# heiheishuang/MuDG

Hardware: AMD Instinct MI355X
Metric: DDIM denoise steps/sec, MDM1024 576x1024x16f (CFG: 2 UNet forwards + fused update per step, per clip) (higher is better)
Workload: dtype bf16; 1 GPU; MDM1024 latents (B=1,4,16,72,128) + c_concat 8ch, context (B,333,1024), 50-step uniform_trailing DDIM schedule, cfg 7.5, guidance_rescale 0.7, eta 1.0, v-prediction, dynamic rescale; clips_per_gpu=1, parallelism=clip-DP x1 (no in-step collective), launch=hipGraph replay of each UNet pass (cond+uncond batched)

## Files before the change

include/mudg_hip.h:

```cpp
#ifndef MUDG_HIP_H
#define MUDG_HIP_H

#include <stdint.h>

#ifdef __cplusplus
extern "C" {
#endif

#define MUDG_OK          0
#define MUDG_EINVAL     -1
#define MUDG_ELAUNCH    -2
#define MUDG_EUNSUPPORTED -3

int mudg_version(void);
int mudg_operand_dtype(void);
const char* mudg_last_error(void);

typedef struct MudgGemmDesc {
    const void* X;
    const void* X2;
    const void* W;
    void*       Y;
    const float* bias;
    const float* gbias;
// ... 3 lines not shown
    int csplit;
    int batch;
    int64_t sX, sW, sY, sR;
    int rows_per_group;
    int out_fp32;
    int res_fp32;
    int geglu;
    int act;
    float alpha;
    int mode;
    int Hin, Win, Hout, Wout, Cin, stride, upsample;
    int pad;
    int korder;
    int T, HW;
    float* stats;
    int subpixel;
    void* Y8; void* S8;
    int ldy8, lds8;
} MudgGemmDesc;
int mudg_gemm(const MudgGemmDesc* d, void* stream);
int mudg_gemm_stats_rows(const MudgGemmDesc* d);
int mudg_conv_subpixel_ok(const MudgGemmDesc* d);
int mudg_gemm_stream_ok(const MudgGemmDesc* d);

typedef struct MudgAttnDesc {
    const void* Q; const void* K; const void* Vt; void* O;
    int F, heads, Nq, Nk;
    int ldq, ldk, ldvt, ldo;
    int64_t svt;
    int kv_div;
    float scale;
    int accumulate;
    const void* K2; const void* Vt2;
    int Nk2, ldk2, ldvt2, kv_div2;
    int64_t svt2;
    const void* Q8; const void* K8; const void* Qs; const void* Ks;
    int ldq8, ldk8, ldqs, ldks;
    int q_prescaled;
    float* Lse;
} MudgAttnDesc;
int mudg_attention(const MudgAttnDesc* d, void* stream);
int mudg_quantize_mxfp8(const void* X, int ldx, int64_t rows, int cols, void* Y8, int ldy, void* S, int lds, void* stream);

int mudg_temporal_attention(const void* QKV, void* O, int B, int T, int HW, int heads,
                            int ldqkv, int ldo, float scale, void* stream);
int mudg_temporal_self_attention_ok(int T, int HW, int heads, int C, int64_t ldx, int64_t ldw, int64_t ldo);
// ... 240 lines not shown
```

mudg_amd/csrc/gemm.hip:

```cpp
#include "gemm_shared.h"
#include <cstdlib>
#include <cmath>
#include <type_traits>

namespace {


template <int NWAVES_, int NI_>
struct Geo {
    static constexpr int NWAVES = NWAVES_, NI = NI_, MI = 2, WN = 2, WM = NWAVES_ / 2;
    static constexpr int NTH = NWAVES * 64;
    static constexpr int BM = WM * MI * 32, BN = WN * NI * 32;
    static constexpr int XI = BM / NWAVES / 8, WI = BN / NWAVES / 8;
    static constexpr int TILE_X = BM * LDSLD, TILE_W = BN * LDSLD;
    static constexpr int STGLD = BN + 4;
    static constexpr bool WIDE = NWAVES > 4;
    static constexpr int WSTRIDE = !WIDE ? NI : (NI & 1 ? 1 : 2);
    static constexpr int nioff(int ni) { return !WIDE ? ni : (NI & 1 ? 2 * ni : 4 * (ni >> 1) + (ni & 1)); }
};
using G128 = Geo<4, 2>;
using G320 = Geo<8, 5>;
using G256 = Geo<8, 4>;

template <typename G> constexpr int stage_elems(bool fast) { return (fused_planes(fast) ? PLANES : 1) * (G::TILE_X + G::TILE_W); }
// ... 722 lines not shown
}
namespace {

template <typename G, int MODE, bool FAST, bool SB = false>
int launch(const MudgGemmDesc& d, int vflags, hipStream_t s) {
    const h16* zp = zero_page();
    if (!zp) MUDG_FAIL(MUDG_ELAUNCH, "gemm: could not allocate the zero page");
    constexpr int smem = smem_main<G>(FAST, SB);
    if (const int rc = mudg_lds_opt_in<&gemm_kernel<G, MODE, FAST, SB>>(smem + PHI_BYTES, "gemm")) return rc;
    const int tiles = ((d.M + G::BM - 1) / G::BM) * ((d.N + G::BN - 1) / G::BN);
    dim3 grid(tiles, 1, d.batch);
    const float* phi = d.geglu ? mudg_phi_table() : nullptr;
    hipLaunchKernelGGL((gemm_kernel<G, MODE, FAST, SB>), grid, dim3(G::NTH), smem + (phi ? PHI_BYTES : 0), s, d, vflags, zp, phi);
    return mudg_check_launch("mudg_gemm");
}

struct GemmSwitches {
    int fast = mudg_variant("GEMM_FAST", 1), sb = mudg_variant("GEMM_SB", 1), persist = mudg_variant("GEMM_PERSIST", 1);
    int wide = mudg_variant("GEMM_WIDE", 2), xshare = mudg_variant("CONV_XSHARE", 1);
    int w288 = mudg_variant("GEMM_W288", 1), w288p = mudg_variant("GEMM_W288P", 1), w288q = mudg_variant("GEMM_W288Q", 0);
    int h144 = mudg_variant("GEMM_H144", 1), h144pf = mudg_variant("GEMM_H144PF", 1);
    int h144delay = mudg_variant("GEMM_H144DELAY", 0) | (mudg_variant("GEMM_H144ABL", 0) << 16) | (mudg_variant("GEMM_H144PRIO", 1) ? 0 : 1 << 20);
    int w160 = mudg_variant("GEMM_W160", 1), w160defer = mudg_variant("GEMM_W160DEFER", 1);
    int stream = mudg_variant("GEMM_STREAM", 1);
};

bool fast_ok(const MudgGemmDesc& d, const GemmSwitches& sw) {
    if (!sw.fast) return false;
    const int cin = d.mode == 0 ? d.K : d.Cin;
    if ((d.K & 63) || (cin & 63) || (d.csplit & 63)) return false;
    if (d.mode == 1 && (d.upsample || d.Hout * d.Wout <= 0)) return false;
    const int64_t ld = d.X2 && d.ldx2 > d.ldx ? d.ldx2 : d.ldx;
    int64_t rel = 255, soff = (int64_t)cin * 2 + (PLANES > 1 ? ld * 2 : 0);
    if (d.mode == 1) {
        rel = (int64_t)(255 / (d.Hout * d.Wout) + 2) * d.Hin * d.Win;
        soff += (int64_t)(2 * d.Win + 2) * ld * 2;
    } else if (d.mode == 2) {
        soff += (int64_t)2 * d.HW * ld * 2;
        if (d.korder) rel = (int64_t)(d.T - 1) * d.HW + 8;
    }
    const int64_t lim = (int64_t)1 << 31;
    return rel * ld * 2 + 128 + soff + 16 < lim && (int64_t)(255 + (PLANES > 1)) * d.ldw * 2 + (int64_t)d.K * 2 + 144 < lim;
}

int access_flags(const MudgGemmDesc& d) {
    int vflags = 0;
    const int ybytes = d.out_fp32 == KIND_F32 ? 4 : 2;
// ... 88 lines not shown

bool wgemm288_ok(const MudgGemmDesc& d, int vflags, const GemmSwitches& sw) {
    if (!sw.w288 || !wgemm_eligible(d, vflags, WBM)) return false;
    if (sw.w288 == 2) return true;
    if (PLANES == 1 && d.geglu && half_height_ok(d, sw)) return true;
    const int S = d.mode == 1 ? d.Hout * d.Wout : d.HW;
    if (S <= 0 || S % WBM != 0) return false;
    if (d.mode != 0 || PLANES == 2) return true;
    if (d.geglu && d.K < 640) return w288_persistent_grid(d, sw) > 0;
    return true;
}

int stream_grid(const MudgGemmDesc& d, int vflags, const GemmSwitches& sw) {
    if (PLANES != 1 || !sw.stream) return 0;
    if (d.mode != 0 || d.K != 320 || (d.N != 320 && d.N != 640) || d.X2 || d.gbias || d.geglu || d.stats) return 0;
    if (sw.stream == 3 && d.N != 320) return 0;
    if (d.out_fp32 == KIND_F32 || (d.R && d.res_fp32 == KIND_F32)) return 0;
    if (!wgemm_eligible(d, vflags, WBM)) return 0;
    if (sw.stream != 2 && !(sw.w288 == 1 && sw.w288p != 2 && sw.w288q != 2 && wgemm288_ok(d, vflags, sw))) return 0;
    const int n = mudg_cu_count(), slices = d.N / 320;
    return n <= 0 ? 0 : ((n < 8 ? 8 : n) / (8 * slices)) * 8 * slices;
}

bool w160_ok(const MudgGemmDesc& d, int vflags, const GemmSwitches& sw) {
    if (!sw.w160 || !wgemm_eligible(d, vflags, QBM)) return false;
    if (sw.w160 == 2) return true;
    const int S = d.mode == 1 ? d.Hout * d.Wout : d.HW;
    if (S <= 0 || S % QBM != 0) return false;
    if (S < 640 || d.geglu) return false;
    if (d.mode != 0) return true;
    return d.K >= 1280;
}

void normalise_desc(MudgGemmDesc& d) {
    if (d.batch < 1) d.batch = 1;
    if (!d.X2) d.csplit = d.mode == 0 ? d.K : d.Cin;
    if (d.alpha == 0.f) d.alpha = 1.f;
}

GemmPlan gemm_plan(const MudgGemmDesc& d) {
    const GemmSwitches sw;
    GemmPlan p{};
    p.vflags = access_flags(d);
    if (d.mode == 2 && d.korder && fast_ok(d, sw)) p.vflags |= VF_TM;
    if (sw.xshare && d.mode == 1 && d.korder && !d.subpixel && !d.upsample && d.stride == 1 && d.pad == 1 && d.Hin == d.Hout && d.Win == d.Wout &&
        d.K == 9 * d.Cin && (d.Cin & 63) == 0)
        p.vflags |= VF_XS;
    p.rows = 128;
    if (const int sg = stream_grid(d, p.vflags, sw); sg > 0) {
        p.rows = WBM;
        p.kernel = GK_STREAM;
        p.grid = sg;
    } else if (PLANES <= 2 && wgemm288_ok(d, p.vflags, sw)) {
        p.rows = WBM;
        if (PLANES == 1 && sw.w288p != 2 && sw.w288q == 2) {
            p.kernel = GK_W288Q;
        } else if (PLANES == 1 && d.geglu && half_height_ok(d, sw)) {
            p.kernel = GK_H144;
            p.pf = sw.h144pf != 0;
            p.delay = sw.h144delay;
        } else if (PLANES == 1 && (p.grid = w288_persistent_grid(d, sw)) > 0) {
            p.kernel = GK_W288P;
        } else {
            p.kernel = GK_W288;
        }
    } else if (PLANES == 1 && w160_ok(d, p.vflags, sw)) {
        p.rows = QBM;
        p.kernel = GK_W160;
        p.rs = !d.R ? 0 : ((d.res_fp32 != KIND_F32 && sw.w160defer) ? 2 : 1);
    } else if (fast_ok(d, sw)) {
        if (PLANES == 1 && (p.ni = use_wide(d, sw)) != 0) {
            p.kernel = GK_WIDE;
        } else if (persistent_ok(d, p.vflags, sw)) {
            p.kernel = GK_PERSIST;
            p.wgs = persistent_wgs(d, sw);
// ... 2 lines not shown
        }
    } else {
        p.kernel = GK_GENERIC;
    }
    return p;
}

}

extern "C" int mudg_gemm_stats_rows(const MudgGemmDesc* dp) {
    if (!dp) return 128;
    MudgGemmDesc d = *dp;
    if (d.out_fp32 < 0 || d.out_fp32 > 2 || d.res_fp32 < 0 || d.res_fp32 > 2 || d.mode < 0 || d.mode > 2) return 128;
    normalise_desc(d);
    return gemm_plan(d).rows;
}

extern "C" int mudg_gemm_stream_ok(const MudgGemmDesc* dp) {
    if (!dp) return 0;
    MudgGemmDesc d = *dp;
    if (d.out_fp32 < 0 || d.out_fp32 > 2 || d.res_fp32 < 0 || d.res_fp32 > 2 || d.mode < 0 || d.mode > 2) return 0;
    normalise_desc(d);
    return gemm_plan(d).kernel == GK_STREAM ? 1 : 0;
}

extern "C" int mudg_conv_subpixel_ok(const MudgGemmDesc* dp) {
    if (!dp) return 0;
    MudgGemmDesc d = *dp;
    if (d.mode != 1 || !d.subpixel || d.batch != 4 || d.stride != 1 || d.pad != 1 || d.upsample || !d.korder) return 0;
    if (d.X2 || d.R || d.gbias || d.stats || d.geglu || d.sX != 0 || d.sY != 0) return 0;
    if (d.Hout != d.Hin || d.Wout != d.Win || d.K != 4 * d.Cin || (d.Cin & 63)) return 0;
    d.csplit = d.Cin;
    return fast_ok(d, GemmSwitches{}) ? 1 : 0;
}

extern "C" int mudg_gemm(const MudgGemmDesc* dp, void* stream) {
    MUDG_REQUIRE(dp, "mudg_gemm: null descriptor");
    MudgGemmDesc d = *dp;
    MUDG_REQUIRE(d.X && d.W && d.Y, "mudg_gemm: null X/W/Y");
    MUDG_REQUIRE(d.M > 0 && d.N > 0 && d.K > 0, "mudg_gemm: empty problem M=%d N=%d K=%d", d.M, d.N, d.K);
    MUDG_REQUIRE(d.mode >= 0 && d.mode <= 2, "mudg_gemm: mode %d", d.mode);
    MUDG_REQUIRE((d.K & 7) == 0, "mudg_gemm: K=%d must be a multiple of 8", d.K);
    MUDG_REQUIRE(d.ldx % (8 * PLANES) == 0 && d.ldw % (8 * PLANES) == 0, "mudg_gemm: ldx=%d ldw=%d must be multiples of %d", d.ldx, d.ldw, 8 * PLANES);
    MUDG_REQUIRE(aligned16(d.X) && aligned16(d.W), "mudg_gemm: X/W must be 16-byte aligned");
    MUDG_REQUIRE((d.sX & 7) == 0 && (d.sW & 7) == 0, "mudg_gemm: batch strides must be multiples of 8");
    normalise_desc(d);
// ... 41 lines not shown
    }
    const GemmPlan plan = gemm_plan(d);
    hipStream_t s = reinterpret_cast<hipStream_t>(stream);
    const int fam = d.mode == 0 ? MUDG_FAM_GEMM : (d.mode == 1 ? MUDG_FAM_CONV : MUDG_FAM_TCONV);
    const int slot = mudg_prof_begin(fam, s);
    int rc = MUDG_EINVAL;
    auto by_mode = [&](auto g, auto fast, auto sb) {
        using G = decltype(g);
        constexpr bool F = decltype(fast)::value, S = decltype(sb)::value;
        const int vf = plan.vflags;
        return d.mode == 0 ? launch<G, 0, F, S>(d, vf, s) : (d.mode == 1 ? launch<G, 1, F, S>(d, vf, s) : launch<G, 2, F, S>(d, vf, s));
    };
    switch (plan.kernel) {
    case GK_GENERIC: rc = by_mode(G128{}, std::false_type{}, std::false_type{}); break;
    case GK_SINGLE: rc = by_mode(G128{}, std::true_type{}, std::true_type{}); break;
#if MUDG_PLANES != 2
    case GK_DOUBLE: rc = by_mode(G128{}, std::true_type{}, std::false_type{}); break;
#endif
#if MUDG_PLANES == 1
    case GK_WIDE: rc = plan.ni == 5 ? by_mode(G320{}, std::true_type{}, std::false_type{}) : by_mode(G256{}, std::true_type{}, std::false_type{}); break;
#endif
    case GK_PERSIST: rc = mudg_pgemm_launch(d, plan, s); break;
    case GK_STREAM: rc = mudg_sgemm_launch(d, plan, s); break;
    default: rc = mudg_wgemm_launch(d, plan, s); break;
    }
    const double flops = 2.0 * d.M * (double)d.N * d.K * d.batch;
    const double nout = d.geglu ? d.N / 2 : d.N;
    double bytes = ((double)d.M * cin + (double)d.N * d.K + (double)d.M * nout * (d.R ? 2.0 : 1.0)) * 2.0 * d.batch;
    if (d.mode == 1 && d.subpixel) bytes = ((double)d.M * cin + 4.0 * d.N * d.K + 4.0 * d.M * nout) * 2.0;
    mudg_prof_end(slot, s, flops, bytes);
    return rc;
}
```

mudg_amd/csrc/gemm_shared.h:

```cpp
#pragma once
#include "common.h"
#include <type_traits>

constexpr int BK = 64;
constexpr int LDSLD = 64;
constexpr int VF_Y = 1, VF_R = 2;
constexpr int VF_TM = 8;
constexpr int VF_XS = 4;

typedef const __attribute__((address_space(1))) void* gptr_t;
typedef __attribute__((address_space(3))) void* lptr_t;

constexpr bool fused_planes(bool fast) { return PLANES == 2 && fast; }

__device__ __forceinline__ float gelu_fast(float x) {
    const float z = fabsf(x) * 0.70710678118654752440f;
    const float t = __frcp_rn(fmaf(0.3275911f, z, 1.0f));
    float p = fmaf(1.061405429f, t, -1.453152027f);
    p = fmaf(p, t, 1.421413741f);
    p = fmaf(p, t, -0.284496736f);
    p = fmaf(p, t, 0.254829592f);
    const float e = 1.0f - p * t * __expf(-z * z);
    return 0.5f * x * (1.0f + copysignf(e, x));
}

constexpr unsigned OOB = 0x80000000u;

__device__ __forceinline__ __amdgpu_buffer_rsrc_t make_rsrc(const h16* base) {
    return __builtin_amdgcn_make_buffer_rsrc(const_cast<h16*>(base), 0, (int)0x80000000u, 0x00020000);
}

constexpr int PHI_N = 1024;
constexpr int PHI_BYTES = (PHI_N + 4) * 4;
__device__ __forceinline__ float gelu_lut(float x, const float* __restrict__ T) {
    float u = fmaf(x, 64.0f, 512.0f);
    u = __builtin_amdgcn_fmed3f(u, 0.0f, 1023.99f);
    const int i = (int)u;
    const float f = u - (float)i;
    const float a = T[i], b = T[i + 1];
    return x * fmaf(f, b - a, a);
}


__device__ __forceinline__ float scale_bias(const float alpha, const float acc, const float bias) { return alpha * acc + bias; }

template <int W>
__device__ __forceinline__ void geglu_gate(float (&v)[W], const float (&gate)[W], const bool phi, const float* __restrict__ phis) {
    if (PLANES > 2) {
#pragma unroll
        for (int j = 0; j < W; ++j) v[j] *= gelu_erf_f(gate[j]);
    } else if (phi) {
#pragma unroll
        for (int j = 0; j < W; ++j) v[j] *= gelu_lut(gate[j], phis);
    } else {
#pragma unroll
        for (int j = 0; j < W; ++j) v[j] *= gelu_fast(gate[j]);
    }
}

template <int W>
__device__ __forceinline__ void stored_value(const float (&v)[W], const int kind, float (&t)[W]) {
    if (kind == KIND_F32) {
#pragma unroll
// ... 188 lines not shown
    w8[0] = mx_pack4_e4m3(r8[0], r8[1], r8[2], r8[3], inv);
    w8[1] = mx_pack4_e4m3(r8[4], r8[5], r8[6], r8[7], inv);
    return w8;
}
#endif


constexpr int WBM = 288, QBM = 160;
constexpr int SBM = 64;
const float* mudg_phi_table(bool split_ok = false);

enum GemmKernel {
    GK_GENERIC,
    GK_DOUBLE,
    GK_SINGLE,
    GK_WIDE,
    GK_PERSIST,
    GK_W288,
    GK_W288P,
    GK_W288Q,
    GK_H144,
    GK_W160,
    GK_STREAM,
};
struct GemmPlan {
    GemmKernel kernel;
    int vflags;
    int rows;
    int ni;
    int wgs;
    int grid;
    int rs;
    bool pf;
    int delay;
};
int mudg_pgemm_launch(const MudgGemmDesc& d, const GemmPlan& plan, hipStream_t s);
int mudg_wgemm_launch(const MudgGemmDesc& d, const GemmPlan& plan, hipStream_t s);
int mudg_sgemm_launch(const MudgGemmDesc& d, const GemmPlan& plan, hipStream_t s);
```

mudg_amd/csrc/sgemm.hip:

```cpp
#include "gemm_shared.h"

#if MUDG_PLANES == 1
namespace {

constexpr int S_C = 320;
constexpr int S_KS = S_C / 32;
constexpr int S_NB = 5;
constexpr int S_RB = SBM / 16;
constexpr int S_TILE = S_RB * S_KS * 1024;
constexpr int S_SLOTS = 3;
constexpr int S_RPIECES = 2 * S_RB + S_RB / 2;
constexpr int S_RWAVE = S_RPIECES * 1024;
constexpr int S_SMEM_X = S_SLOTS * S_TILE, S_SMEM_R = 4 * S_RWAVE;
static_assert(S_RB == 4, "wave w stages row block w");
static_assert(S_SMEM_X + S_SMEM_R <= 160 * 1024, "LDS");
constexpr int X_DMA = S_KS, R_DMA = S_RPIECES, STORES = 2 * S_RB + S_RB / 2;
static_assert(X_DMA == 10 && STORES == 10 && R_DMA == 10, "S_WAIT_FIRST / S_WAIT_TILE below are X_DMA and X_DMA + STORES");
#define S_WAIT_FIRST() asm volatile("s_waitcnt vmcnt(10)" ::: "memory")
#define S_WAIT_TILE() asm volatile("s_waitcnt vmcnt(20)" ::: "memory")
#define S_LGKM0() asm volatile("s_waitcnt lgkmcnt(0)" ::: "memory")
#define S_BARRIER()                            \
    do {                                       \
        __builtin_amdgcn_sched_barrier(0);     \
        __builtin_amdgcn_s_barrier();          \
        __builtin_amdgcn_sched_barrier(0);     \
    } while (0)

__device__ __forceinline__ f32x4 s_mfma(h16x8 a, h16x8 b, f32x4 c) {
#ifdef MUDG_OPERAND_FP16
    return __builtin_amdgcn_mfma_f32_16x16x32_f16(a, b, c, 0, 0, 0);
#else
    return __builtin_amdgcn_mfma_f32_16x16x32_bf16(a, b, c, 0, 0, 0);
#endif
}

template <bool HASR, bool RF16, bool YF16>
__global__ __launch_bounds__(256, 1) void sgemm_kernel(const MudgGemmDesc p, const int ntiles, const int nslices) {
    extern __shared__ __attribute__((aligned(1024))) char smem[];
    const int tid = threadIdx.x, lane = tid & 63;
    const int wave = __builtin_amdgcn_readfirstlane(tid >> 6);
    const int xcd = blockIdx.x & 7, idx = blockIdx.x >> 3;
    const int slice = idx % nslices, wg = (idx / nslices) * 8 + xcd, nwg = (int)gridDim.x / nslices;
    const int per = ntiles / nwg, rem = ntiles % nwg;
    const int t0 = wg * per + (wg < rem ? wg : rem), t1 = t0 + per + (wg < rem ? 1 : 0);
    if (t0 == t1) return;

    const int px = lane & 15, q4 = lane >> 4;
    const int n0 = S_C * slice;
    const int cpair = n0 + 64 * wave + 8 * q4;
    const int csingle = n0 + 256 + 16 * wave;

    const int pos = lane * 16;
    const int sbyte = pos ^ (((pos >> 9) & 1) << 5);
    const int srow = sbyte >> 6, schunk = (sbyte >> 4) & 3;
    const h16* X = reinterpret_cast<const h16*>(p.X);
    const unsigned vx = (unsigned)(srow * p.ldx) * 2u + (unsigned)schunk * 16u;
    const int xrow = 16 * wave + srow;
    const int xsoff = 16 * wave * p.ldx * 2;
    char* const xdst = smem + wave * S_KS * 1024;
    auto issue_x = [&](const int t, const int slot) {
        const int64_t m0 = (int64_t)t * SBM;
        const bool live = t < t1 && m0 + xrow < p.M;
        const __amdgpu_buffer_rsrc_t rX = make_rsrc(X + m0 * p.ldx);
        const unsigned v = live ? vx : OOB;
        char* d = xdst + slot * S_TILE;
#pragma unroll
        for (int s = 0; s < S_KS; ++s) __builtin_amdgcn_raw_ptr_buffer_load_lds(rX, (lptr_t)(d + s * 1024), 16, (int)v, xsoff + s * 64, 0, 0);
    };
    const int hrow = px + 16 * (q4 & 1), hcol = csingle + 8 * (q4 >> 1);
    char* const rdst = smem + S_SMEM_X + wave * S_RWAVE;
    const h16* R = reinterpret_cast<const h16*>(p.R);
    const unsigned vrp = HASR ? (unsigned)(px * p.ldr + cpair) * 2u : 0u, vrs = HASR ? (unsigned)(hrow * p.ldr + hcol) * 2u : 0u;
    auto issue_r = [&](const int t) {
        const int64_t m0 = (int64_t)t * SBM;
        const int64_t lim = t < t1 ? p.M : 0;
        const __amdgpu_buffer_rsrc_t rR = make_rsrc(R + m0 * p.ldr);
#pragma unroll
        for (int i = 0; i < S_RB; ++i) {
            const bool live = m0 + 16 * i + px < lim;
#pragma unroll
            for (int P = 0; P < 2; ++P)
                __builtin_amdgcn_raw_ptr_buffer_load_lds(rR, (lptr_t)(rdst + (2 * i + P) * 1024), 16, (int)(live ? vrp + 64u * P : OOB), i * 16 * p.ldr * 2, 0, 0);
        }
#pragma unroll
        for (int u = 0; u < S_RB / 2; ++u) {
            const bool live = m0 + 32 * u + hrow < lim;
            __builtin_amdgcn_raw_ptr_buffer_load_lds(rR, (lptr_t)(rdst + (2 * S_RB + u) * 1024), 16, (int)(live ? vrs : OOB), u * 32 * p.ldr * 2, 0, 0);
        }
    };
    auto seed = [&](f32x4 (&acc)[S_RB][S_NB]) {
        u32x4 ra[S_RB][2];
// ... 117 lines not shown
            }
            u32x4 bits;
#pragma unroll
            for (int d = 0; d < 2; ++d) {
                const auto sw = __builtin_amdgcn_permlane16_swap(h[0][d], h[1][d], false, false);
                bits[d] = sw[0]; bits[2 + d] = sw[1];
            }
            const bool live = m0 + 32 * u + hrow < p.M;
            __builtin_amdgcn_raw_buffer_store_b128(bits, rY, (int)(live ? vys : OOB), u * 32 * p.ldy * 2, 0);
        }
        slot = slot == 2 ? 0 : slot + 1;
    }
}

template <bool HASR, bool RF16, bool YF16>
int sgemm_launch(const MudgGemmDesc& d, int grid, hipStream_t s) {
    constexpr int smem = S_SMEM_X + (HASR ? S_SMEM_R : 0);
    if (const int rc = mudg_lds_opt_in<&sgemm_kernel<HASR, RF16, YF16>>(smem, "gemm")) return rc;
    const int ntiles = (d.M + SBM - 1) / SBM;
    hipLaunchKernelGGL((sgemm_kernel<HASR, RF16, YF16>), dim3(grid), dim3(256), smem, s, d, ntiles, d.N / S_C);
    return mudg_check_launch("mudg_gemm");
}

}

int mudg_sgemm_launch(const MudgGemmDesc& d, const GemmPlan& plan, hipStream_t s) {
    if (plan.grid <= 0 || d.N % S_C != 0 || plan.grid % (8 * (d.N / S_C)) != 0 || d.out_fp32 == KIND_F32 || (d.R && d.res_fp32 == KIND_F32)) MUDG_FAIL(MUDG_EINVAL, "gemm: not a problem of the stream kernel");
    const bool yf = d.out_fp32 == KIND_F16, rf = d.res_fp32 == KIND_F16;
    if (!d.R) return yf ? sgemm_launch<false, false, true>(d, plan.grid, s) : sgemm_launch<false, false, false>(d, plan.grid, s);
    if (rf) return yf ? sgemm_launch<true, true, true>(d, plan.grid, s) : sgemm_launch<true, true, false>(d, plan.grid, s);
    return yf ? sgemm_launch<true, false, true>(d, plan.grid, s) : sgemm_launch<true, false, false>(d, plan.grid, s);
}
#else
int mudg_sgemm_launch(const MudgGemmDesc&, const GemmPlan&, hipStream_t) { MUDG_FAIL(MUDG_EINVAL, "gemm: no stream kernel in this build"); }
#endif
```

mudg_amd/csrc/wgemm.hip:

```cpp
#include "gemm_shared.h"
#include <type_traits>

#if MUDG_PLANES <= 2
namespace {

constexpr int WNA = WBM / 16;
constexpr int W_TAIL = 2 * 320 * 2 * 4;
constexpr int W_TAIL_GEGLU = (PHI_N + 4) * 8;
template <int NREP> struct WGeo {
    static constexpr int BN = 64 * NREP;
    static constexpr int NB = BN / 16;
    static constexpr int PL = (WNA + NB) * 1024;
    static constexpr int KS = PLANES * PL;
    static constexpr int BUF = 2 * KS;
    static constexpr int LOOP = (4 / PLANES) * KS;
    static constexpr int SMEM = LOOP + (NREP == 4 ? W_TAIL_GEGLU : W_TAIL);
};

#define W_BARRIER()                            \
    do {                                       \
        __builtin_amdgcn_sched_barrier(0);     \
        __builtin_amdgcn_s_barrier();          \
        __builtin_amdgcn_sched_barrier(0);     \
    } while (0)
#define W_VMCNT(n) asm volatile("s_waitcnt vmcnt(" #n ")" ::: "memory")
#ifdef MUDG_DEBUG_VARIANTS
[[maybe_unused]] __device__ unsigned long long* g_stamps = nullptr;
#define W_STAMP(slot) do { if (tid == 0 && g_stamps && (slot) < 64) g_stamps[(size_t)blockIdx.x * 64 + (slot)] = __builtin_amdgcn_s_memtime(); } while (0)
#else
#define W_STAMP(slot) do { } while (0)
#endif
// ... 6 lines not shown
    return __builtin_amdgcn_mfma_f32_16x16x32_bf16(a, b, c, 0, 0, 0);
#endif
}
__device__ __forceinline__ void mfma16_inplace(h16x8 a, h16x8 b, f32x4& c) {
#ifdef MUDG_OPERAND_FP16
    asm volatile("v_mfma_f32_16x16x32_f16 %0, %1, %2, %0" : "+v"(c) : "v"(a), "v"(b));
#else
    asm volatile("v_mfma_f32_16x16x32_bf16 %0, %1, %2, %0" : "+v"(c) : "v"(a), "v"(b));
#endif
}
__device__ __forceinline__ unsigned opaque(unsigned v) { asm volatile("" : "+v"(v)); return v; }
template <int CTRL>
__device__ __forceinline__ float dpp_add16(float v) {
    return v + __int_as_float(__builtin_amdgcn_update_dpp(0, __float_as_int(v), CTRL, 0xf, 0xf, false));
}
__device__ __forceinline__ float row16_sum(float v) {
    v = dpp_add16<0xB1>(v);
    v = dpp_add16<0x4E>(v);
    v = dpp_add16<0x141>(v);
    v = dpp_add16<0x140>(v);
    return v;
}

__device__ __forceinline__ float gelu_lut2(float x, const f32x2* __restrict__ T) {
    float u = fmaf(x, 64.0f, 512.0f);
    u = __builtin_amdgcn_fmed3f(u, 0.0f, 1023.99f);
    const f32x2 t = T[(int)u];
    return x * fmaf(__builtin_amdgcn_fractf(u), t[1], t[0]);
}
__device__ __forceinline__ float gelu_hermite(float x, const f32x2* __restrict__ T) {
    float u = fmaf(x, 64.0f, 512.0f);
    u = __builtin_amdgcn_fmed3f(u, 0.0f, 1023.99f);
    const int i = (int)u;
    const float t = __builtin_amdgcn_fractf(u);
    const f32x2 n0 = T[i], n1 = T[i + 1];
    const float dl = n1[0] - n0[0];
    const float c3 = fmaf(-2.0f, dl, n0[1] + n1[1]);
    const float c2 = dl - n0[1] - c3;
    float r = fmaf(t, c3, c2);
    r = fmaf(t, r, n0[1]);
    r = fmaf(t, r, n0[0]);
    return x * r;
}
template <int NREP> __device__ __forceinline__ int wave_pair_col(int wc, int pair) { return 32 * ((NREP / 2) * wc + pair); }
template <int NREP> __device__ __forceinline__ int wave_single_col(int wc) { return 32 * (NREP / 2) * 4 + 16 * wc; }

template <int NREP, int NI>
__device__ __forceinline__ void w_seed(const MudgGemmDesc& p, f32x4 (&acc)[NI][NREP], const int m0, const int n0, const int wr, const int wc, const int lane) {
    constexpr int NPAIR = NREP / 2;
    const int px = lane & 15, q4 = lane >> 4;
    const int RK = p.res_fp32;
    const int64_t mrow = (int64_t)m0 + wr * (16 * NI) + px;
// ... 101 lines not shown
#pragma unroll
        for (int e = 0; e < 8; ++e) { gs[e] = 0.f; gq[e] = 0.f; }
#pragma unroll
        for (int i = 0; i < NI; ++i) {
            const int64_t m = mrow + 16 * i;
            const bool live = m < p.M;
            float v[8];
            if constexpr (GEGLU) {
                float val[8], gate[8];
#pragma unroll
                for (int e = 0; e < 8; ++e) {
                    const float a = acc[i][e >> 2][e & 3], b = acc[i][2 + (e >> 2)][e & 3];
                    val[e] = UA ? a + bv[e] : scale_bias(alpha, a, bv[e]);
                    gate[e] = UA ? b + bg[e] : scale_bias(alpha, b, bg[e]);
                }
                if constexpr (!TAB || (PLANES != 2 && LUT == 1)) {
#pragma unroll
                    for (int e = 0; e < 8; ++e) v[e] = val[e];
                    geglu_gate<8>(v, gate, TAB, tail);
                } else if constexpr (PLANES == 2) {
#pragma unroll
                    for (int e = 0; e < 8; ++e) v[e] = val[e] * gelu_hermite(gate[e], phis);
                } else {
                    float u[8];
                    f32x2 t[8];
#pragma unroll
                    for (int e = 0; e < 8; ++e) u[e] = __builtin_amdgcn_fmed3f(fmaf(gate[e], 64.0f, 512.0f), 0.0f, 1023.99f);
#pragma unroll
                    for (int e = 0; e < 8; ++e) t[e] = phis[(int)u[e]];
#pragma unroll
                    for (int e = 0; e < 8; ++e) v[e] = val[e] * (gate[e] * fmaf(__builtin_amdgcn_fractf(u[e]), t[e][1], t[e][0]));
                }
            } else {
#pragma unroll
                for (int e = 0; e < 8; ++e) {
                    const float a = acc[i][2 * P + (e >> 2)][e & 3];
                    v[e] = UA ? a + bv[e] : scale_bias(alpha, a, bv[e]);
                }
                if constexpr (DR) add_residual_raw(v, sraw[i][P], zero16(), decltype(rtag)::value == 1 ? KIND_F16 : KIND_OPERAND);
            }
            if (!GEGLU && p.stats) {
                float t[8];
                stored_value(v, OK, t);
                stats_add(t, live ? 8 : 0, gs, gq);
            }
            if (live) store_piece(p.Y, m * p.ldy + n, OK, p.ldy / PLANES, v, 8, true);
        }
        if (!GEGLU && p.stats) {
#pragma unroll
            for (int e = 0; e < 8; ++e) { gs[e] = row16_sum(gs[e]); gq[e] = row16_sum(gq[e]); }
            if (px == 0) {
                float* d = sred + ((wr * WBN) + wave_pair_col<NREP>(wc, P) + 8 * q4) * 2;
#pragma unroll
                for (int e = 0; e < 8; ++e) { d[2 * e] = gs[e]; d[2 * e + 1] = gq[e]; }
// ... 1220 lines not shown
```

mudg_amd/hip.py:

```python
from __future__ import annotations

import ctypes as C
import os

_HERE = os.path.dirname(os.path.abspath(__file__))
LIB_PATHS = {"bf16": os.path.join(_HERE, "libmudg_hip.so"), "fp16": os.path.join(_HERE, "libmudg_hip_fp16.so"),
             "bf16x3": os.path.join(_HERE, "libmudg_hip_x3.so"), "bf16x6": os.path.join(_HERE, "libmudg_hip_x6.so")}
_MODES = {"bf16": (0, 1), "fp16": (1, 1), "bf16x3": (2, 2), "bf16x6": (3, 3)}
_operand = os.environ.get("MUDG_OPERAND", "bf16").lower()
LIB_PATH = LIB_PATHS["bf16"]


def set_operand(name: str) -> None:
    global _operand
    name = name.lower()
    if name not in LIB_PATHS:
        raise MudgError(f"unknown operand type {name!r} ({' | '.join(LIB_PATHS)})")
    if _lib is not None and name != _operand:
        raise MudgError("the operand type must be chosen before the first kernel call")
    _operand = name


def operand_name() -> str:
    return _operand
# ... 73 lines not shown
        ("T", C.c_int), ("HW", C.c_int),
        ("slices", C.c_int), ("chunk", C.c_int64),
    ]


class ShortAttnDesc(C.Structure):
    _fields_ = [
        ("QKV", C.c_void_p), ("O", C.c_void_p),
        ("B", C.c_int), ("heads", C.c_int), ("N", C.c_int), ("d", C.c_int),
        ("ldqkv", C.c_int64), ("ldo", C.c_int64),
        ("scale", C.c_float),
    ]


_P, _I, _L, _F, _D = C.c_void_p, C.c_int, C.c_int64, C.c_float, C.c_double
SIGNATURES = {
    "mudg_version": (_I, []),
    "mudg_operand_dtype": (_I, []),
    "mudg_last_error": (C.c_char_p, []),
    "mudg_gemm": (_I, [C.POINTER(GemmDesc), _P]),
    "mudg_gemm_stats_rows": (_I, [C.POINTER(GemmDesc)]),
    "mudg_conv_subpixel_ok": (_I, [C.POINTER(GemmDesc)]),
    "mudg_gemm_stream_ok": (_I, [C.POINTER(GemmDesc)]),
    "mudg_attention": (_I, [C.POINTER(AttnDesc), _P]),
    "mudg_quantize_mxfp8": (_I, [_P, _I, _L, _I, _P, _I, _P, _I, _P]),
    "mudg_temporal_attention": (_I, [_P, _P, _I, _I, _I, _I, _I, _I, _F, _P]),
    "mudg_temporal_self_attention_ok": (_I, [_I, _I, _I, _I, _L, _L, _L]),
    "mudg_temporal_self_attention": (_I, [_P, _P, _P, _I, _I, _I, _I, _I, _L, _L, _L, _F, _P]),
    "mudg_groupnorm_ws_floats": (_L, [_I, _I, _I]),
    "mudg_groupnorm": (_I, [_P, _P, _I, _I, _I, _I, _P, _P, _P, _I, _I, _I, _I, _I, _F, _I, _P, _P]),
    "mudg_groupnorm_fused": (_I, [_P, _P, _I, _I, _I, _I, _P, _P, _P, _I, _I, _I, _I, _I, _F, _I, _P, _P, _P, _P]),
    "mudg_groupnorm_fused_rows": (_I, [_P, _P, _I, _I, _I, _I, _P, _P, _P, _I, _I, _I, _I, _I, _F, _I, _P, _I, _P, _I, _P, _P]),
    "mudg_layernorm": (_I, [_P, _I, _I, _P, _P, _P, _I, _I, _I, _F, _P]),
    "mudg_softmax_rows": (_I, [_P, _I, _P, _I, _I, _I, _P]),
    "mudg_timestep_embedding": (_I, [_P, _P, _P, _I, _I, _P]),
    "mudg_small_linear": (_I, [_P, _P, _I, _P, _P, _I, _I, _I, _I, _I, _I, _P]),
    "mudg_ncthw_to_rows": (_I, [_P, _I, _P, _I, _I, _I, _I, _I, _I, _I, _I, _P]),
    "mudg_rows_to_ncthw": (_I, [_P, _I, _I, _I, _P, _I, _I, _I, _I, _I, _F, _I, _I, _P]),
    "mudg_cast_f32_bf16": (_I, [_P, _P, _L, _P]),
    "mudg_cast_rows": (_I, [_P, _I, _L, _P, _I, _L, _L, _L, _P]),
    "mudg_zero_channels": (_I, [_P, _I, _I, _I, _I, _P]),
    "mudg_copy_rows": (_I, [_P, _L, _P, _L, _L, _L, _P]),
    "mudg_axpy_f32": (_I, [_P, _P, _L, _F, _P]),
    "mudg_lincomb": (_I, [_P, _P, _P, _P, _P, _I, _L, _P]),
    "mudg_ddim_ws_doubles": (_L, [_I]),
    "mudg_frames_to_u8": (_I, [_P, _P, _I, _I, _I, _L, _P]),
# ... 143 lines not shown
```

Baseline: 8.536 steps/s.

## Add persistent streaming GEGLU GEMM kernel for K=320 feed-forward projections

Adds a persistent, XCD-aware streaming GEMM kernel specialised for the K=320 GEGLU feed-forward input projection. It keeps the weights in registers, streams X tiles into LDS via buffer-load-to-LDS with triple buffering, and software-pipelines the LUT-based GELU epilogue of the previous row block under the MFMAs of the next. It is meant to cut the memory- and epilogue-bound time of the largest-resolution GEGLU layers. It is only selected for large M (at least 9216 rows) with the default switch settings, and it adds register pressure and hand-tuned waitcnt assumptions.

New measurement: 8.618 steps/s, median of 6. About the same (+1.0%).

```diff
diff --git a/include/mudg_hip.h b/include/mudg_hip.h
--- a/include/mudg_hip.h
+++ b/include/mudg_hip.h
@@ -49,6 +49,7 @@
 int mudg_gemm_stats_rows(const MudgGemmDesc* d);
 int mudg_conv_subpixel_ok(const MudgGemmDesc* d);
 int mudg_gemm_stream_ok(const MudgGemmDesc* d);
+int mudg_gemm_stream_geglu_ok(const MudgGemmDesc* d);
 
 typedef struct MudgAttnDesc {
     const void* Q; const void* K; const void* Vt; void* O;
diff --git a/mudg_amd/csrc/gemm.hip b/mudg_amd/csrc/gemm.hip
--- a/mudg_amd/csrc/gemm.hip
+++ b/mudg_amd/csrc/gemm.hip
@@ -768,7 +768,8 @@
     int h144 = mudg_variant("GEMM_H144", 1), h144pf = mudg_variant("GEMM_H144PF", 1);
     int h144delay = mudg_variant("GEMM_H144DELAY", 0) | (mudg_variant("GEMM_H144ABL", 0) << 16) | (mudg_variant("GEMM_H144PRIO", 1) ? 0 : 1 << 20);
     int w160 = mudg_variant("GEMM_W160", 1), w160defer = mudg_variant("GEMM_W160DEFER", 1);
-    int stream = mudg_variant("GEMM_STREAM", 1);
+    int stream = mudg_variant("GEMM_STREAM", 1), stream_geglu = mudg_variant("GEMM_STREAM_GEGLU", 1);
+    int gelu_lut = mudg_variant("GELU_LUT", 1);
 };
 
 bool fast_ok(const MudgGemmDesc& d, const GemmSwitches& sw) {
@@ -903,6 +904,22 @@
     return n <= 0 ? 0 : ((n < 8 ? 8 : n) / (8 * slices)) * 8 * slices;
 }
 
+constexpr int STREAM_GEGLU_MIN_ROWS = 9216;
+int stream_geglu_grid(const MudgGemmDesc& d, int vflags, const GemmSwitches& sw) {
+    if (PLANES != 1 || !sw.stream_geglu || !sw.gelu_lut) return 0;
+    if (!d.geglu || d.mode != 0 || d.K != 320 || d.N % 256 != 0 || d.X2 || d.out_fp32 == KIND_F32) return 0;
+    if (!wgemm_eligible(d, vflags, WBM)) return 0;
+    const int n = mudg_cu_count(), slices = d.N / 256;
+    if (n <= 0) return 0;
+    const int cus = (n < 8 ? 8 : n) & ~7;
+    if (slices > cus / 8) return 0;
+    if (sw.stream_geglu != 2) {
+        if (!(sw.fast == 1 && sw.persist == 1 && sw.wide == 2 && sw.w288 == 1 && sw.w288p == 1 && sw.w288q == 0 && sw.h144 == 1)) return 0;
+        if (d.M < STREAM_GEGLU_MIN_ROWS) return 0;
+    }
+    return (cus / (8 * slices)) * 8 * slices;
+}
+
 bool w160_ok(const MudgGemmDesc& d, int vflags, const GemmSwitches& sw) {
     if (!sw.w160 || !wgemm_eligible(d, vflags, QBM)) return false;
     if (sw.w160 == 2) return true;
@@ -932,6 +949,9 @@
         p.rows = WBM;
         p.kernel = GK_STREAM;
         p.grid = sg;
+    } else if (const int gg = stream_geglu_grid(d, p.vflags, sw); gg > 0) {
+        p.kernel = GK_STREAM_GEGLU;
+        p.grid = gg;
     } else if (PLANES <= 2 && wgemm288_ok(d, p.vflags, sw)) {
         p.rows = WBM;
         if (PLANES == 1 && sw.w288p != 2 && sw.w288q == 2) {
@@ -980,6 +1000,14 @@
     if (d.out_fp32 < 0 || d.out_fp32 > 2 || d.res_fp32 < 0 || d.res_fp32 > 2 || d.mode < 0 || d.mode > 2) return 0;
     normalise_desc(d);
     return gemm_plan(d).kernel == GK_STREAM ? 1 : 0;
+}
+
+extern "C" int mudg_gemm_stream_geglu_ok(const MudgGemmDesc* dp) {
+    if (!dp) return 0;
+    MudgGemmDesc d = *dp;
+    if (d.out_fp32 < 0 || d.out_fp32 > 2 || d.res_fp32 < 0 || d.res_fp32 > 2 || d.mode < 0 || d.mode > 2) return 0;
+    normalise_desc(d);
+    return gemm_plan(d).kernel == GK_STREAM_GEGLU ? 1 : 0;
 }
 
 extern "C" int mudg_conv_subpixel_ok(const MudgGemmDesc* dp) {
@@ -1067,6 +1095,7 @@
 #endif
     case GK_PERSIST: rc = mudg_pgemm_launch(d, plan, s); break;
     case GK_STREAM: rc = mudg_sgemm_launch(d, plan, s); break;
+    case GK_STREAM_GEGLU: rc = mudg_sgeglu_launch(d, plan, s); break;
     default: rc = mudg_wgemm_launch(d, plan, s); break;
     }
     const double flops = 2.0 * d.M * (double)d.N * d.K * d.batch;
diff --git a/mudg_amd/csrc/gemm_shared.h b/mudg_amd/csrc/gemm_shared.h
--- a/mudg_amd/csrc/gemm_shared.h
+++ b/mudg_amd/csrc/gemm_shared.h
@@ -39,6 +39,23 @@
     const float f = u - (float)i;
     const float a = T[i], b = T[i + 1];
     return x * fmaf(f, b - a, a);
+}
+constexpr int PHI_PAIR_BYTES = (PHI_N + 4) * 8;
+__device__ __forceinline__ float lut2_pos(float x) { return __builtin_amdgcn_fmed3f(fmaf(x, 64.0f, 512.0f), 0.0f, 1023.99f); }
+__device__ __forceinline__ float lut2_gelu(float x, float u, f32x2 t) { return x * fmaf(__builtin_amdgcn_fractf(u), t[1], t[0]); }
+__device__ __forceinline__ float gelu_lut2(float x, const f32x2* __restrict__ T) {
+    const float u = lut2_pos(x);
+    return lut2_gelu(x, u, T[(int)u]);
+}
+__device__ __forceinline__ void geglu_lut2_piece(float (&v)[8], const float (&val)[8], const float (&gate)[8], const f32x2* __restrict__ T) {
+    float u[8];
+    f32x2 t[8];
+#pragma unroll
+    for (int e = 0; e < 8; ++e) u[e] = lut2_pos(gate[e]);
+#pragma unroll
+    for (int e = 0; e < 8; ++e) t[e] = T[(int)u[e]];
+#pragma unroll
+    for (int e = 0; e < 8; ++e) v[e] = val[e] * lut2_gelu(gate[e], u[e], t[e]);
 }
 
 
@@ -273,6 +290,7 @@
     GK_H144,
     GK_W160,
     GK_STREAM,
+    GK_STREAM_GEGLU,
 };
 struct GemmPlan {
     GemmKernel kernel;
@@ -288,3 +306,4 @@
 int mudg_pgemm_launch(const MudgGemmDesc& d, const GemmPlan& plan, hipStream_t s);
 int mudg_wgemm_launch(const MudgGemmDesc& d, const GemmPlan& plan, hipStream_t s);
 int mudg_sgemm_launch(const MudgGemmDesc& d, const GemmPlan& plan, hipStream_t s);
+int mudg_sgeglu_launch(const MudgGemmDesc& d, const GemmPlan& plan, hipStream_t s);
diff --git a/mudg_amd/csrc/sgemm.hip b/mudg_amd/csrc/sgemm.hip
--- a/mudg_amd/csrc/sgemm.hip
+++ b/mudg_amd/csrc/sgemm.hip
@@ -34,39 +34,61 @@
 #endif
 }
 
+struct SRange { int slice, t0, t1; };
+__device__ __forceinline__ SRange s_range(const int ntiles, const int nslices) {
+    const int xcd = blockIdx.x & 7, idx = blockIdx.x >> 3;
+    const int slice = idx % nslices, wg = (idx / nslices) * 8 + xcd, nwg = (int)gridDim.x / nslices;
+    const int per = ntiles / nwg, rem = ntiles % nwg;
+    const int t0 = wg * per + (wg < rem ? wg : rem);
+    return SRange{slice, t0, t0 + per + (wg < rem ? 1 : 0)};
+}
+
+struct SXStage {
+    const h16* X;
+    char* xdst;
+    unsigned vx;
+    int xrow, xsoff, ldx, M, t1;
+    __device__ __forceinline__ SXStage(const MudgGemmDesc& p, char* smem, const int wave, const int lane, const int t1_)
+        : X(reinterpret_cast<const h16*>(p.X)), xdst(smem + wave * S_KS * 1024), ldx(p.ldx), M(p.M), t1(t1_) {
+        const int pos = lane * 16;
+        const int sbyte = pos ^ (((pos >> 9) & 1) << 5);
+        const int srow = sbyte >> 6, schunk = (sbyte >> 4) & 3;
+        vx = (unsigned)(srow * p.ldx) * 2u + (unsigned)schunk * 16u;
+        xrow = 16 * wave + srow;
+        xsoff = 16 * wave * p.ldx * 2;
+    }
+    struct Tile { __amdgpu_buffer_rsrc_t rX; unsigned v; char* d; };
+    __device__ __forceinline__ Tile tile(const int t, const int slot) const {
+        const int64_t m0 = (int64_t)t * SBM;
+        const bool live = t < t1 && m0 + xrow < M;
+        return Tile{make_rsrc(X + m0 * ldx), live ? vx : OOB, xdst + slot * S_TILE};
+    }
+    __device__ __forceinline__ void piece(const Tile& x, const int s) const {
+        __builtin_amdgcn_raw_ptr_buffer_load_lds(x.rX, (lptr_t)(x.d + s * 1024), 16, (int)x.v, xsoff + s * 64, 0, 0);
+    }
+    __device__ __forceinline__ void issue(const int t, const int slot) const {
+        const Tile x = tile(t, slot);
+#pragma unroll
+        for (int s = 0; s < S_KS; ++s) piece(x, s);
+    }
+};
+
 template <bool HASR, bool RF16, bool YF16>
 __global__ __launch_bounds__(256, 1) void sgemm_kernel(const MudgGemmDesc p, const int ntiles, const int nslices) {
     extern __shared__ __attribute__((aligned(1024))) char smem[];
     const int tid = threadIdx.x, lane = tid & 63;
     const int wave = __builtin_amdgcn_readfirstlane(tid >> 6);
-    const int xcd = blockIdx.x & 7, idx = blockIdx.x >> 3;
-    const int slice = idx % nslices, wg = (idx / nslices) * 8 + xcd, nwg = (int)gridDim.x / nslices;
-    const int per = ntiles / nwg, rem = ntiles % nwg;
-    const int t0 = wg * per + (wg < rem ? wg : rem), t1 = t0 + per + (wg < rem ? 1 : 0);
+    const SRange rg = s_range(ntiles, nslices);
+    const int t0 = rg.t0, t1 = rg.t1;
     if (t0 == t1) return;
 
     const int px = lane & 15, q4 = lane >> 4;
-    const int n0 = S_C * slice;
+    const int n0 = S_C * rg.slice;
     const int cpair = n0 + 64 * wave + 8 * q4;
     const int csingle = n0 + 256 + 16 * wave;
 
-    const int pos = lane * 16;
-    const int sbyte = pos ^ (((pos >> 9) & 1) << 5);
-    const int srow = sbyte >> 6, schunk = (sbyte >> 4) & 3;
-    const h16* X = reinterpret_cast<const h16*>(p.X);
-    const unsigned vx = (unsigned)(srow * p.ldx) * 2u + (unsigned)schunk * 16u;
-    const int xrow = 16 * wave + srow;
-    const int xsoff = 16 * wave * p.ldx * 2;
-    char* const xdst = smem + wave * S_KS * 1024;
-    auto issue_x = [&](const int t, const int slot) {
-        const int64_t m0 = (int64_t)t * SBM;
-        const bool live = t < t1 && m0 + xrow < p.M;
-        const __amdgpu_buffer_rsrc_t rX = make_rsrc(X + m0 * p.ldx);
-        const unsigned v = live ? vx : OOB;
-        char* d = xdst + slot * S_TILE;
-#pragma unroll
-        for (int s = 0; s < S_KS; ++s) __builtin_amdgcn_raw_ptr_buffer_load_lds(rX, (lptr_t)(d + s * 1024), 16, (int)v, xsoff + s * 64, 0, 0);
-    };
+    const SXStage xst(p, smem, wave, lane, t1);
+    auto issue_x = [&](const int t, const int slot) { xst.issue(t, slot); };
     const int hrow = px + 16 * (q4 & 1), hcol = csingle + 8 * (q4 >> 1);
     char* const rdst = smem + S_SMEM_X + wave * S_RWAVE;
     const h16* R = reinterpret_cast<const h16*>(p.R);
@@ -230,6 +252,162 @@
     return mudg_check_launch("mudg_gemm");
 }
 
+constexpr int G_NB = 4;
+constexpr int G_SLICE = 64 * S_RB;
+constexpr int G_STORES = S_RB;
+constexpr int G_AHEAD = 4;
+constexpr int G_SMEM = S_SMEM_X + PHI_PAIR_BYTES;
+static_assert(G_SMEM <= 160 * 1024, "LDS");
+static_assert(X_DMA == 10 && G_STORES == 4, "G_WAIT_TILE below is G_STORES + X_DMA + G_STORES; a range's first tile waits S_WAIT_FIRST");
+#define G_WAIT_TILE() asm volatile("s_waitcnt vmcnt(18)" ::: "memory")
+
+template <bool UA, bool YF16>
+__global__ __launch_bounds__(256, 1) void sgeglu_kernel(const MudgGemmDesc p, const float* __restrict__ phi, const int ntiles, const int nslices) {
+    extern __shared__ __attribute__((aligned(1024))) char smem[];
+    const int tid = threadIdx.x, lane = tid & 63;
+    const int wave = __builtin_amdgcn_readfirstlane(tid >> 6);
+    const SRange rg = s_range(ntiles, nslices);
+    const int t0 = rg.t0, t1 = rg.t1;
+    if (t0 == t1) return;
+
+    const int px = lane & 15, q4 = lane >> 4;
+    const int n0 = G_SLICE * rg.slice;
+    const int cw = n0 + 64 * wave + 8 * q4;
+    const int nout = (n0 >> 1) + 32 * wave + 8 * q4;
+
+    const SXStage xst(p, smem, wave, lane, t1);
+    const int fbyte0 = px * 64 + q4 * 16;
+    const int fbyte = fbyte0 ^ (((fbyte0 >> 9) & 1) << 5);
+    const float alpha = p.alpha;
+    h16* Y = reinterpret_cast<h16*>(p.Y);
+    const unsigned vy = (unsigned)(px * p.ldy + nout) * 2u;
+    f32x2* const phis = reinterpret_cast<f32x2*>(smem + S_SMEM_X);
+
+    xst.issue(t0, 0);
+    xst.issue(t0 + 1, 1);
+
+    h16x8 wf[G_NB][S_KS];
+    {
+        const h16* W = reinterpret_cast<const h16*>(p.W);
+#pragma unroll
+        for (int j = 0; j < G_NB; ++j) {
+            const int ch = n0 + 64 * wave + 32 * (j >> 1) + 8 * (px >> 2) + 4 * (j & 1) + (px & 3);
+            const h16* wrow = W + (int64_t)ch * p.ldw + 8 * q4;
+#pragma unroll
+            for (int s = 0; s < S_KS; ++s) wf[j][s] = as_h16x8(ld16(wrow + 32 * s));
+        }
+    }
+    float bv[8] = {}, bg[8] = {};
+    if (p.bias) {
+#pragma unroll
+        for (int e = 0; e < 8; ++e) { bv[e] = p.bias[cw + e]; bg[e] = p.bias[cw + 32 + e]; }
+    }
+    for (int t = tid; t <= PHI_N; t += 256) {
+        const float a = phi[t], b = phi[t < PHI_N ? t + 1 : t];
+        phis[t] = f32x2{a, b - a};
+    }
+    S_LGKM0();
+#pragma unroll
+    for (int j = 0; j < G_NB; ++j)
+#pragma unroll
+        for (int s = 0; s < S_KS; ++s) asm volatile("" : "+v"(wf[j][s]));
+
+    struct Epi { float val[8], gate[8], u[8], v[8]; f32x2 t[8]; };
+    using T0 = std::integral_constant<int, 0>; using T1 = std::integral_constant<int, 1>; using T2 = std::integral_constant<int, 2>;
+    using T3 = std::integral_constant<int, 3>; using TN = std::integral_constant<int, -1>;
+    SXStage::Tile xnext{};
+    auto block = [&](auto itag, const char* xs, h16x8 (&xf)[S_RB * S_KS], f32x4 (&am)[G_NB], const f32x4 (&ae)[G_NB], const int64_t m0e, const int ie)
+                     __attribute__((always_inline)) {
+        constexpr int I = decltype(itag)::value;
+        constexpr bool MMA = I >= 0;
+        Epi E;
+#pragma unroll
+        for (int s = 0; s < S_KS; ++s) {
+            if constexpr (I == 0) xst.piece(xnext, s);
+            if constexpr (MMA) {
+                constexpr int Q = I < 0 ? 0 : I * S_KS;
+                if (Q + s + G_AHEAD < S_RB * S_KS) xf[Q + s + G_AHEAD] = *reinterpret_cast<const h16x8*>(xs + (Q + s + G_AHEAD) * 1024);
+#pragma unroll
+                for (int j = 0; j < G_NB; ++j) am[j] = s_mfma(wf[j][s], xf[Q + s], am[j]);
+            }
+            if (s < 8) {
+                const int e = s;
+                float a = ae[e >> 2][e & 3], b = ae[2 + (e >> 2)][e & 3];
+                asm volatile("" : "+v"(a));
+                E.val[e] = UA ? a + bv[e] : scale_bias(alpha, a, bv[e]);
+                asm volatile("" : "+v"(b), "+v"(E.val[e]));
+                E.gate[e] = UA ? b + bg[e] : scale_bias(alpha, b, bg[e]);
+                E.u[e] = lut2_pos(E.gate[e]);
+                E.t[e] = phis[(int)E.u[e]];
+            }
+            if (s >= 2) {
+                const int e = s - 2;
+                E.v[e] = E.val[e] * lut2_gelu(E.gate[e], E.u[e], E.t[e]);
+                asm volatile("" : "+v"(E.v[e]));
+            }
+            __builtin_amdgcn_sched_barrier(0);
+        }
+        const u32x4 bits = YF16 ? f16_bits(E.v) : operand_bits(E.v);
+        const bool live = m0e + 16 * ie + px < p.M;
+        __builtin_amdgcn_raw_buffer_store_b128(bits, make_rsrc(Y + m0e * p.ldy), (int)(live ? vy : OOB), ie * 16 * p.ldy * 2, 0);
+        __builtin_amdgcn_sched_barrier(0);
+    };
+
+    f32x4 acc3[G_NB];
+#pragma unroll
+    for (int j = 0; j < G_NB; ++j) acc3[j] = f32x4{0.f, 0.f, 0.f, 0.f};
+    int64_t m0p = p.M;
+    int slot = 0;
+    for (int t = t0; t < t1; ++t) {
+        if (t == t0) S_WAIT_FIRST(); else G_WAIT_TILE();
+        S_BARRIER();
+        const char* xs = smem + slot * S_TILE + fbyte;
+        h16x8 xf[S_RB * S_KS];
+#pragma unroll
+        for (int s = 0; s < G_AHEAD; ++s) xf[s] = *reinterpret_cast<const h16x8*>(xs + s * 1024);
+        f32x4 acc[S_RB - 1][G_NB];
+#pragma unroll
+        for (int i = 0; i < S_RB - 1; ++i)
+#pragma unroll
+            for (int j = 0; j < G_NB; ++j) acc[i][j] = f32x4{0.f, 0.f, 0.f, 0.f};
+        xnext = xst.tile(t + 2, slot == 0 ? 2 : slot - 1);
+        __builtin_amdgcn_sched_barrier(0);
+
+        const int64_t m0 = (int64_t)t * SBM;
+        block(T0{}, xs, xf, acc[0], acc3, m0p, 3);
+#pragma unroll
+        for (int j = 0; j < G_NB; ++j) acc3[j] = f32x4{0.f, 0.f, 0.f, 0.f};
+        block(T1{}, xs, xf, acc[1], acc[0], m0, 0);
+        block(T2{}, xs, xf, acc[2], acc[1], m0, 1);
+        block(T3{}, xs, xf, acc3, acc[2], m0, 2);
+        m0p = m0;
+        slot = slot == 2 ? 0 : slot + 1;
+    }
+    {
+        h16x8 none[S_RB * S_KS];
+        f32x4 unused[G_NB];
+        block(TN{}, nullptr, none, unused, acc3, m0p, 3);
+    }
+}
+
+template <bool UA, bool YF16>
+int sgeglu_launch(const MudgGemmDesc& d, const float* phi, int grid, hipStream_t s) {
+    if (const int rc = mudg_lds_opt_in<&sgeglu_kernel<UA, YF16>>(G_SMEM, "gemm")) return rc;
+    const int ntiles = (d.M + SBM - 1) / SBM;
+    hipLaunchKernelGGL((sgeglu_kernel<UA, YF16>), dim3(grid), dim3(256), G_SMEM, s, d, phi, ntiles, d.N / G_SLICE);
+    return mudg_check_launch("mudg_gemm");
+}
+
+}
+
+int mudg_sgeglu_launch(const MudgGemmDesc& d, const GemmPlan& plan, hipStream_t s) {
+    if (plan.grid <= 0 || !d.geglu || d.K != S_C || d.N % G_SLICE != 0 || plan.grid % (8 * (d.N / G_SLICE)) != 0 || d.out_fp32 == KIND_F32 || d.R)
+        MUDG_FAIL(MUDG_EINVAL, "gemm: not a problem of the stream GEGLU kernel");
+    const float* phi = mudg_phi_table(false);
+    if (!phi) MUDG_FAIL(MUDG_ELAUNCH, "gemm: the stream GEGLU kernel needs the Phi table");
+    const bool yf = d.out_fp32 == KIND_F16;
+    if (d.alpha == 1.f) return yf ? sgeglu_launch<true, true>(d, phi, plan.grid, s) : sgeglu_launch<true, false>(d, phi, plan.grid, s);
+    return yf ? sgeglu_launch<false, true>(d, phi, plan.grid, s) : sgeglu_launch<false, false>(d, phi, plan.grid, s);
 }
 
 int mudg_sgemm_launch(const MudgGemmDesc& d, const GemmPlan& plan, hipStream_t s) {
@@ -241,4 +419,5 @@
 }
 #else
 int mudg_sgemm_launch(const MudgGemmDesc&, const GemmPlan&, hipStream_t) { MUDG_FAIL(MUDG_EINVAL, "gemm: no stream kernel in this build"); }
+int mudg_sgeglu_launch(const MudgGemmDesc&, const GemmPlan&, hipStream_t) { MUDG_FAIL(MUDG_EINVAL, "gemm: no stream GEGLU kernel in this build"); }
 #endif
diff --git a/mudg_amd/csrc/wgemm.hip b/mudg_amd/csrc/wgemm.hip
--- a/mudg_amd/csrc/wgemm.hip
+++ b/mudg_amd/csrc/wgemm.hip
@@ -6,7 +6,7 @@
 
 constexpr int WNA = WBM / 16;
 constexpr int W_TAIL = 2 * 320 * 2 * 4;
-constexpr int W_TAIL_GEGLU = (PHI_N + 4) * 8;
+constexpr int W_TAIL_GEGLU = PHI_PAIR_BYTES;
 template <int NREP> struct WGeo {
     static constexpr int BN = 64 * NREP;
     static constexpr int NB = BN / 16;
@@ -59,12 +59,6 @@
     return v;
 }
 
-__device__ __forceinline__ float gelu_lut2(float x, const f32x2* __restrict__ T) {
-    float u = fmaf(x, 64.0f, 512.0f);
-    u = __builtin_amdgcn_fmed3f(u, 0.0f, 1023.99f);
-    const f32x2 t = T[(int)u];
-    return x * fmaf(__builtin_amdgcn_fractf(u), t[1], t[0]);
-}
 __device__ __forceinline__ float gelu_hermite(float x, const f32x2* __restrict__ T) {
     float u = fmaf(x, 64.0f, 512.0f);
     u = __builtin_amdgcn_fmed3f(u, 0.0f, 1023.99f);
@@ -212,14 +206,7 @@
 #pragma unroll
                     for (int e = 0; e < 8; ++e) v[e] = val[e] * gelu_hermite(gate[e], phis);
                 } else {
-                    float u[8];
-                    f32x2 t[8];
-#pragma unroll
-                    for (int e = 0; e < 8; ++e) u[e] = __builtin_amdgcn_fmed3f(fmaf(gate[e], 64.0f, 512.0f), 0.0f, 1023.99f);
-#pragma unroll
-                    for (int e = 0; e < 8; ++e) t[e] = phis[(int)u[e]];
-#pragma unroll
-                    for (int e = 0; e < 8; ++e) v[e] = val[e] * (gate[e] * fmaf(__builtin_amdgcn_fractf(u[e]), t[e][1], t[e][0]));
+                    geglu_lut2_piece(v, val, gate, phis);
                 }
             } else {
 #pragma unroll
diff --git a/mudg_amd/hip.py b/mudg_amd/hip.py
--- a/mudg_amd/hip.py
+++ b/mudg_amd/hip.py
@@ -119,6 +119,7 @@
     "mudg_gemm_stats_rows": (_I, [C.POINTER(GemmDesc)]),
     "mudg_conv_subpixel_ok": (_I, [C.POINTER(GemmDesc)]),
     "mudg_gemm_stream_ok": (_I, [C.POINTER(GemmDesc)]),
+    "mudg_gemm_stream_geglu_ok": (_I, [C.POINTER(GemmDesc)]),
     "mudg_attention": (_I, [C.POINTER(AttnDesc), _P]),
     "mudg_quantize_mxfp8": (_I, [_P, _I, _L, _I, _P, _I, _P, _I, _P]),
     "mudg_temporal_attention": (_I, [_P, _P, _I, _I, _I, _I, _I, _I, _F, _P]),
```
